# hibikid39/ndt_slam

Hardware: AMD Instinct MI355X
Metric: scan-matches/sec (10k-pt scan vs 1M-pt NDT map) (higher is better)
Workload: dtype f64

## Files before the change

### include/ndt_mi355x.h

```cpp
#ifndef NDT_MI355X_H_
#define NDT_MI355X_H_

#include <stddef.h>
#include <stdint.h>

#ifdef __cplusplus
extern "C" {
#endif

enum ndt_status {
  NDT_OK = 0,
  NDT_E_ARG = -1,
  NDT_E_HIP = -2,
  NDT_E_NO_DEVICE = -3,
  NDT_E_GRID = -4,
  NDT_E_NOMEM = -5
};

typedef struct ndt_params {
  float  resolution;
  double step_size;
  double trans_eps;
  int    max_iter;
  double outlier_ratio;
// ... 25 lines not shown
  int    evals;
  int    ref_evals;
  int    converged;
  int    status;
  int    flags;
  double kbar;
} ndt_result;

enum ndt_result_flags {
  NDT_FLAG_WINDOW_SPILL  = 1,
  NDT_FLAG_REGION_CLIPPED = 2,
  NDT_FLAG_UNSORTED      = 4
};

typedef struct ndt_map_info {
  int min_bx, min_by, div_x, div_y;
  int n_cells;
  int n_valid;
  size_t n_points;
} ndt_map_info;

typedef struct ndt_ctx ndt_ctx;
typedef struct ndt_map ndt_map;

int ndt_default_params(ndt_params *p);
int ndt_params_pcl110(ndt_params *p);
int ndt_params_pcl18(ndt_params *p);
int ndt_params_pcl_new(ndt_params *p);

int ndt_ctx_create(int device, ndt_ctx **out);
int ndt_ctx_destroy(ndt_ctx *ctx);
const char *ndt_last_error(const ndt_ctx *ctx);
void *ndt_ctx_stream(ndt_ctx *ctx);
enum ndt_option { NDT_OPT_MAX_HELPERS = 1, NDT_OPT_WORKGROUPS = 2, NDT_OPT_INJECT_FAULT = 3, NDT_OPT_DEFER_FITNESS = 4 };
int ndt_ctx_set_option(ndt_ctx *ctx, int option, long long value);
int ndt_ctx_set_stream(ndt_ctx *ctx, void *stream);

int ndt_map_build(ndt_ctx *ctx, const float *xy_host, size_t n, size_t stride_bytes,
                  const ndt_params *prm, ndt_map **map);
int ndt_map_build_dev(ndt_ctx *ctx, const float *xy_dev, size_t n, size_t stride_bytes,
                      const ndt_params *prm, ndt_map **map);
#define NDT_REBUILT 1
int ndt_map_rebuild_begin(ndt_ctx *ctx, const float *xy_dev, size_t n, size_t stride_bytes,
                          const ndt_params *prm, ndt_map *map);
int ndt_map_rebuild_end(ndt_ctx *ctx, ndt_map *map);
int ndt_map_destroy(ndt_map *map);
int ndt_map_info_get(const ndt_map *map, ndt_map_info *out);
int ndt_map_export(const ndt_map *map, int *cell_idx, float *cent_xy, double *mean_xy,
                   double *icov_xx_xy_yy, int *npts);

int ndt_align(ndt_ctx *ctx, const ndt_map *map, const float *scan_xy_host, size_t n,
              size_t stride_bytes, const double init_xyyaw[3], ndt_result *out);

int ndt_align_batch(ndt_ctx *ctx, const ndt_map *map, const float *scans_xy_host,
                    const uint64_t *offsets_host, int B, int shared_scan,
                    const double *inits_host , ndt_result *out_host );
int ndt_align_batch_dev(ndt_ctx *ctx, const ndt_map *map, const float *scans_xy_dev,
                        const uint64_t *offsets_dev, int B, size_t total_points, int shared_scan,
                        const double *inits_dev, ndt_result *out_dev, void *stream);
int ndt_align_batch_prepare_dev(ndt_ctx *ctx, const ndt_map *map, const float *scans_xy_dev,
                                const uint64_t *offsets_dev, int B, size_t total_points, int shared_scan,
                                const double *inits_dev, void *stream);
int ndt_prepare_timing(ndt_ctx *ctx, float *order_ms);

int ndt_align_batch_sharded(ndt_ctx *const *ctxs, const ndt_map *const *maps, int n_shards, const float *scans_xy_host,
                            const uint64_t *offsets, int B, int shared_scan, const double *inits_xyyaw,
                            ndt_result *results);
// ... 66 lines not shown
```

### ndt_slam_amd/capi.py

```python
import ctypes as C
import os
import sys

import numpy as np

_HERE = os.path.dirname(os.path.abspath(__file__))
LIB_PATH = os.environ.get("NDT_LIB_PATH") or os.path.join(_HERE, "libndt_mi355x.so")
_LIB = None


class NdtError(RuntimeError):
    pass


class Params(C.Structure):
    _fields_ = [
        ("resolution", C.c_float), ("step_size", C.c_double), ("trans_eps", C.c_double),
        ("max_iter", C.c_int), ("outlier_ratio", C.c_double), ("min_pts", C.c_int),
        ("eig_mult", C.c_double), ("cov_unbiased", C.c_int), ("cov_init_identity", C.c_int),
        ("conv_ge", C.c_int), ("radius_inclusive", C.c_int), ("transform_sse", C.c_int),
        ("stale_h_ang", C.c_int), ("snap_thresh", C.c_double), ("mt_max_iter", C.c_int),
        ("mt_mu", C.c_double), ("mt_nu", C.c_double), ("libm_f32", C.c_int), ("grid_margin", C.c_int),
    ]


class FuseParams(C.Structure):
    _fields_ = [("coe_ndt_cov", C.c_double), ("coe_vel", C.c_double), ("coe_omega", C.c_double),
                ("del_time", C.c_double), ("score_thre", C.c_double)]


class MapInfo(C.Structure):
    _fields_ = [("min_bx", C.c_int), ("min_by", C.c_int), ("div_x", C.c_int), ("div_y", C.c_int),
                ("n_cells", C.c_int), ("n_valid", C.c_int), ("n_points", C.c_size_t)]


RESULT_DTYPE = np.dtype([
    ("pose", "f8", 3), ("T00", "f4"), ("T10", "f4"), ("T03", "f4"), ("T13", "f4"),
    ("fitness", "f8"), ("trans_prob", "f8"), ("score", "f8"), ("H", "f8", 9), ("p", "f8", 3),
    ("iters", "i4"), ("evals", "i4"), ("ref_evals", "i4"), ("converged", "i4"), ("status", "i4"),
    ("flags", "i4"), ("kbar", "f8")], align=True)
RESULT_BYTES = RESULT_DTYPE.itemsize
FLAG_WINDOW_SPILL, FLAG_REGION_CLIPPED, FLAG_UNSORTED = 1, 2, 4
NDT_OK, NDT_E_ARG, NDT_E_HIP, NDT_E_NO_DEVICE, NDT_E_GRID, NDT_E_NOMEM = 0, -1, -2, -3, -4, -5
OPT_MAX_HELPERS, OPT_WORKGROUPS, OPT_INJECT_FAULT, OPT_DEFER_FITNESS = 1, 2, 3, 4

EXPORTS = [
    "ndt_default_params", "ndt_params_pcl110", "ndt_params_pcl18", "ndt_params_pcl_new", "ndt_ctx_create", "ndt_ctx_destroy", "ndt_last_error", "ndt_ctx_stream",
    "ndt_ctx_set_stream", "ndt_ctx_set_option", "ndt_ctx_wait_launch",
    "ndt_map_build", "ndt_map_build_dev", "ndt_map_rebuild_begin", "ndt_map_rebuild_end", "ndt_map_destroy", "ndt_map_info_get", "ndt_map_export",
    "ndt_align", "ndt_align_batch", "ndt_align_batch_dev", "ndt_align_batch_prepare_dev", "ndt_prepare_timing", "ndt_align_batch_trace", "ndt_eval_at",
    "ndt_fitness_at", "ndt_last_timing", "ndt_kernel_timing", "ndt_launch_interval", "ndt_align_batch_sharded", "ndt_prefilter", "ndt_prefilter_batch_dev",
    "ndt_fuse_default_params", "ndt_predict_batch_dev", "ndt_fuse_batch_dev",
    "ndt_remove_neighbors", "ndt_remove_neighbors_dev",
    "ndt_difference_extraction", "ndt_difference_extraction_dev", "ndt_make_map", "ndt_make_map_dev",
    "ndt_selftest_libm_f32",
]


def lib():
    global _LIB
    if _LIB is not None:
        return _LIB
    if not os.path.exists(LIB_PATH):
        raise NdtError("%s is missing: run `python -c 'import __graft_entry__ as g; g.build()'` "
                       "(hipcc --offload-arch=gfx950); there is no CPU fallback" % LIB_PATH)
    L = C.CDLL(LIB_PATH)
    vp, sz, i = C.c_void_p, C.c_size_t, C.c_int
    for name in ("ndt_default_params", "ndt_params_pcl110", "ndt_params_pcl18", "ndt_params_pcl_new"):
        getattr(L, name).argtypes = [C.POINTER(Params)]
    L.ndt_ctx_create.argtypes = [i, C.POINTER(vp)]
    L.ndt_ctx_destroy.argtypes = [vp]
    L.ndt_last_error.restype = C.c_char_p
    L.ndt_last_error.argtypes = [vp]
    L.ndt_ctx_stream.restype = vp
    L.ndt_ctx_stream.argtypes = [vp]
    L.ndt_ctx_set_stream.argtypes = [vp, vp]
    L.ndt_ctx_set_option.argtypes = [vp, i, C.c_longlong]
# ... 325 lines not shown
```

### ndt_slam_amd/csrc/ndt_match.hip.h

```cpp

constexpr int kBlock = 1024;
constexpr int kWaves = kBlock / 64;
#ifndef NDT_KSUB
#define NDT_KSUB 4
#endif
constexpr int kSub = NDT_KSUB;
constexpr int kUnits = kWaves * kSub;
#ifndef NDT_MAX_HELPERS_BUILD
#define NDT_MAX_HELPERS_BUILD 15
#endif
constexpr int kMaxHelpers = NDT_MAX_HELPERS_BUILD;
constexpr int kDefaultHelpers = 8;
constexpr int kBatchHelpers = 2;
#ifndef NDT_IDLE_MAX
#define NDT_IDLE_MAX 800
#endif
#ifndef NDT_XCD_BONUS
#define NDT_XCD_BONUS 6
#endif
#ifndef NDT_NEED_SLOPE
#define NDT_NEED_SLOPE 10
#endif
#ifndef NDT_HELPER_PENALTY
#define NDT_HELPER_PENALTY 12
// ... 98 lines not shown
  int sbox[4];
  int swave[kWaves + 1];
  int sflag[4];
  double wpart[kUnits * 12];
  double wtmp[kWaves * 12];
  double tot[12];
  unsigned long long own_mask;
  unsigned long long hpose[8];
  unsigned long long hword;
  int hrank;
  int jnext;
  int steal;
  unsigned diag[2];
  int clipped;
  MapView M;
  OptParams P;
  const float2 *pts;
  int npts;
  double etab[64];
};

__shared__ Lds g_L;
__shared__ uint4 g_pool[kPoolBytes / 16];

__device__ __forceinline__ Window window_of(const Region &R, const uint4 *pool) {
  Window W;
  W.R = R;
  W.slot = reinterpret_cast<const unsigned short *>(pool);
  W.ent = reinterpret_cast<const CellEntry *>(reinterpret_cast<const char *>(pool) +
                                              ((R.rw * R.rh * 2 + 15) / 16) * 16);
  return W;
}

__device__ __forceinline__ void region_from_bbox(const MapView &M, const Tf32 &T0, Lds &L) {
  {
    Region r = {0, 0, 0, 0, 0, 0};
    L.clipped = 0;
    if (L.sbox[0] <= L.sbox[2]) {
      long long x0 = (long long)L.sbox[0] - kRegionMargin, x1 = (long long)L.sbox[2] + kRegionMargin;
      long long y0 = (long long)L.sbox[1] - kRegionMargin, y1 = (long long)L.sbox[3] + kRegionMargin;
      long long w = x1 - x0 + 1, h = y1 - y0 + 1;
      if (w > 0 && h > 0) {
        if (w * h > kRegionCells) {
          L.clipped = 1;
          const long long w2 = w > 128 ? 128 : w;
          long long h2 = kRegionCells / w2; if (h2 > h) h2 = h;
          const float sx = fminf(fmaxf(floorf(T0.tx * M.inv_leaf), -1.0e9f), 1.0e9f);
          const float sy = fminf(fmaxf(floorf(T0.ty * M.inv_leaf), -1.0e9f), 1.0e9f);
          long long cx0 = ((long long)(int)sx - M.min_bx) - w2 / 2, cy0 = ((long long)(int)sy - M.min_by) - h2 / 2;
          cx0 = cx0 < x0 ? x0 : (cx0 > x1 - w2 + 1 ? x1 - w2 + 1 : cx0);
          cy0 = cy0 < y0 ? y0 : (cy0 > y1 - h2 + 1 ? y1 - h2 + 1 : cy0);
          x0 = cx0; y0 = cy0; w = w2; h = h2;
        }
        const long long far = 1ll << 30;
        x0 = x0 < -far ? -far : (x0 > far ? far : x0); y0 = y0 < -far ? -far : (y0 > far ? far : y0);
        r.x0 = (int)x0; r.y0 = (int)y0; r.rw = (int)w; r.rh = (int)h;
      }
    }
    const int slot_bytes = ((r.rw * r.rh * 2 + 15) / 16) * 16;
    int cap = (kPoolBytes - slot_bytes) / (int)sizeof(CellEntry) - 2;
    r.cap = cap > 0xFFF0 ? 0xFFF0 : cap;
    L.RG = r;
  }
}

template <bool SSE>
__device__ __noinline__ void compute_region(const MapView &M, const Tf32 &T0, const float2 *__restrict__ scan,
// ... 627 lines not shown
    for (; q < q1; ++q) {
      if (lane < 12) dst[(q - q0) * dst_stride + lane] = 0.0;
    }
    if (step != 0 && vtot) {
      const int u = q0 * kWaves + w;
      __builtin_amdgcn_fence(__ATOMIC_RELEASE, "wavefront");
      __builtin_amdgcn_wave_barrier();
      __builtin_amdgcn_fence(__ATOMIC_ACQUIRE, "wavefront");
      if (lane < kUnitWords) {
        const u64 bits = (u64)__double_as_longlong(dst[lane >> 1]);
        st64(&vtot[u * kUnitWords + lane], tag | (u64)(u32)((lane & 1) ? (bits >> 32) : bits));
      }
    }
  }
}

__device__ __forceinline__ bool watchdog(WsHeader *hdr, u64 spin_start, unsigned &polls) {
  if ((++polls & 63u) != 0u) return false;
  if (ld32(&hdr->abort)) return true;
  if (wall_clock64() - spin_start > kWatchTicks) { st32(&hdr->abort, 1u); return true; }
  return false;
}

__device__ __forceinline__ u64 wave_bcast64(u64 v) {
  const u32 lo = __builtin_amdgcn_readfirstlane((u32)v), hi = __builtin_amdgcn_readfirstlane((u32)(v >> 32));
  return ((u64)hi << 32) | lo;
}

struct alignas(16) PrepRec {
  int region[6];
  int clipped, ok;
  AlignState S;
};
constexpr int kPrepWords = (int)(sizeof(PrepRec) / 4);
static_assert(sizeof(PrepRec) % 16 == 0 && kPrepWords <= kBlock, "PrepRec is copied word by word by one workgroup");

template <bool SSE>
__global__ void __launch_bounds__(kBlock)
ndt_order_kernel(MapView M, OptParams P, const float *__restrict__ scans, const unsigned long long *__restrict__ offsets,
                 int B, int shared_scan, const double *__restrict__ inits, float2 *__restrict__ sorted,
                 PrepRec *__restrict__ prep, unsigned *__restrict__ prep_map ) {
  Lds &L = g_L;
  uint4 *const pool = g_pool;
  if (threadIdx.x == 64) { L.M = M; L.P = P; }
  __syncthreads();
  for (int b = (int)blockIdx.x; b < B; b += (int)gridDim.x) {
    const u64 o0 = shared_scan ? offsets[0] : offsets[b];
    const u64 o1 = shared_scan ? offsets[1] : offsets[b + 1];
    const int n = (int)(o1 - o0);
    PrepRec *R = prep + b;
    if (!(n > 0 && n <= kSortRegs)) {
      if (threadIdx.x == 0) R->ok = 0;
      continue;
    }
    const float2 *scan = reinterpret_cast<const float2 *>(scans) + o0;
    float2 *sp = shared_scan ? sorted + (size_t)b * (size_t)n : sorted + o0;
    order_scan_regs<SSE, kSortRegs / kBlock>(L.M, L.P, inits + 3 * (size_t)b, scan, n, L, pool, sp);
    copy_out_ordered(pool, sp, n);
    if (threadIdx.x == 0) {
      const Region r = L.RG;
      R->region[0] = r.x0; R->region[1] = r.y0; R->region[2] = r.rw; R->region[3] = r.rh; R->region[4] = r.cap; R->region[5] = 0;
      R->clipped = L.clipped; R->ok = 1;
    }
    {
      const u32 *src = reinterpret_cast<const u32 *>(&L.S);
      u32 *dst = reinterpret_cast<u32 *>(&R->S);
      if (threadIdx.x < sizeof(AlignState) / 4) dst[threadIdx.x] = src[threadIdx.x];
      const unsigned *wmap = reinterpret_cast<const unsigned *>(L.wpart);
      unsigned *gm = prep_map + (size_t)b * (kRegionCells / 32);
      for (int i = threadIdx.x; i < kRegionCells / 32; i += kBlock) gm[i] = wmap[i];
    }
    __syncthreads();
  }
}

template <bool SSE, bool INCL, bool CHK>
__global__ void __launch_bounds__(kBlock)
ndt_align_kernel(MapView M, OptParams P, const float *__restrict__ scans,
                 const unsigned long long *__restrict__ offsets, int B, int shared_scan,
                 const double *__restrict__ inits, ndt_result *__restrict__ results,
                 double *__restrict__ trace, int trace_cap, int *__restrict__ trace_rows,
                 float2 *__restrict__ sorted ,
                 unsigned char *__restrict__ ws ,
                 int allow_helpers ,
                 unsigned long long *__restrict__ prof ,
                 const PrepRec *__restrict__ prep ,
                 const unsigned *__restrict__ prep_map) {
  Lds &L = g_L;
  uint4 *const pool = g_pool;
  WsHeader *hdr = reinterpret_cast<WsHeader *>(ws);
  ScanCtl *ctl = reinterpret_cast<ScanCtl *>(ws + sizeof(WsHeader));
  u64 *utot = reinterpret_cast<u64 *>(ws + sizeof(WsHeader) + (size_t)B * sizeof(ScanCtl));
  unsigned *wantmap = reinterpret_cast<unsigned *>(ws + sizeof(WsHeader) + (size_t)B * sizeof(ScanCtl) +
                                                  (size_t)B * kUnits * kUnitWords * sizeof(u64));
  const u64 t_start = kProf ? wall_clock64() : 0;
  const int lane = threadIdx.x & 63, wave = threadIdx.x >> 6;
  if (threadIdx.x < 64) L.etab[threadIdx.x] = c_exp2_tab[threadIdx.x];
  if (threadIdx.x == 64) { L.M = M; L.P = P; }
  bool aborted = false;

  int preclaimed = -1;
  int b0 = (int)blockIdx.x;
  if (allow_helpers && B > 0 && B < (int)gridDim.x && blockIdx.x < 4u * (unsigned)B)
// ... 479 lines not shown
```

### ndt_slam_amd/csrc/ndt_mi355x.hip

```cpp

#include <hip/hip_runtime.h>
#include <hip/hip_ext.h>

#include <algorithm>
#include <cfloat>
#include <cmath>
#include <cstdio>
#include <cstdlib>
#include <cstring>
#include <new>
#include <string>
#include <mutex>
#include <set>
#include <utility>
#include <vector>

#include "ndt_mi355x.h"

#pragma clang fp contract(off)

namespace {

thread_local std::string g_last_error;

// ... 86 lines not shown
  PinnedBuf<unsigned> h_bounds;
  std::string err;
  float map_ms = 0.f, align_ms = 0.f;
  DevBuf<unsigned char> d_scan, d_tmp;
  DevBuf<uint64_t> d_off;
  DevBuf<double> d_init, d_trace;
  DevBuf<ndt_result> d_res;
  DevBuf<int> d_rows;
  DevBuf<float> d_fit;
  DevBuf<FitPart> d_fit_part;
  DevBuf<unsigned char> d_far;
  DevBuf<unsigned char> d_pf;
  DevBuf<unsigned char> d_rn;
  DevBuf<unsigned char> d_mm;
  PinnedBuf<unsigned char> h_mm;
  hipEvent_t ev_mm = nullptr; bool mm_pending = false;
  int num_cus = 0;
  int helpers = -1;
  int workgroups = 0;
  int inject_fault = 0;
  struct PrepSet {
    DevBuf<float2> sorted;
    DevBuf<PrepRec> recs;
    DevBuf<unsigned char> maps;
    hipEvent_t ev0 = nullptr, ready = nullptr;
    bool valid = false, timed = false;
    const void *scans = nullptr, *offsets = nullptr, *inits = nullptr, *map = nullptr;
    int B = 0, shared_scan = 0; size_t total_points = 0;
    int min_bx = 0, min_by = 0, div_x = 0, div_y = 0; float inv_leaf = 0.f;
    long long reader = -1;
  } prep[2];
  int prep_last = 1;
  float order_ms = 0.f;
  hipEvent_t ev_scratch = nullptr; hipStream_t scratch_stream = nullptr; bool scratch_used = false, scratch_recorded = false;
  struct LaunchSet { DevBuf<unsigned char> ws; DevBuf<float2> sorted; size_t ws_clean = 0; };
  static constexpr int kDeferSets = 2;
  LaunchSet sets[kDeferSets];
  LaunchRing ring;
  int defer_fitness = 0;
  hipStream_t fit_stream = nullptr;
  struct FitJob {
    MapView V; const float *scans = nullptr; const unsigned long long *offsets = nullptr; int B = 0, shared_scan = 0;
    size_t total_points = 0; float2 *sorted = nullptr; ndt_result *out = nullptr; unsigned char *ws = nullptr;
    size_t zero_bytes = 0, far_cnt_bytes = 0; bool sse = false; hipEvent_t end = nullptr;
  };
  bool deferred_pending = false;
};

struct ndt_map {
  ndt_ctx *ctx = nullptr;
  ndt_params prm;
  ndt_map_info info;
  bool info_valid = false;
  MapView view;
  size_t n = 0, ng = 0, npad = 0;
  DevBuf<int> count, start, npts_grid;
  DevBuf<unsigned long long> scan_state;
  unsigned scan_seq = 0;
  bool count_clean = false;
  DevBuf<int> perm;
  DevBuf<float2> pts, cent;
  DevBuf<double> rec;
  DevBuf<unsigned> bounds; DevBuf<int> counters;
  DevBuf<int> big;
  DevBuf<unsigned> occ;
  DevBuf<unsigned long long> tiles;
  bool pending = false, pend_queued = false;
  const float *pend_xy = nullptr; size_t pend_stride = 0;
  GridDims grid; bool have_grid = false;
  DevBuf<unsigned char> xy_stage;
  std::vector<std::pair<ndt_ctx *, unsigned long long>> readers;
};

namespace {

int fail(ndt_ctx *ctx, int code, const std::string &msg) {
  g_last_error = msg;
  if (ctx) ctx->err = msg;
  return code;
}

struct ScratchScope {
  ndt_ctx *ctx; hipStream_t st; bool is_open = false;
  ScratchScope(ndt_ctx *c, hipStream_t s) : ctx(c), st(s) {}
  ScratchScope(const ScratchScope &) = delete;
  ScratchScope &operator=(const ScratchScope &) = delete;
  int open(bool deferred_launch = false) {
    if (ctx->deferred_pending && !deferred_launch && ctx->ring.launches > 0) {
      HIP_TRY(ctx, hipStreamWaitEvent(st, ctx->ring.end(ctx->ring.launches - 1), 0));
      ctx->deferred_pending = false;
    }
    if (ctx->scratch_used && st != ctx->scratch_stream) {
      if (!ctx->scratch_recorded) HIP_TRY(ctx, hipEventRecord(ctx->ev_scratch, ctx->scratch_stream));
      HIP_TRY(ctx, hipStreamWaitEvent(st, ctx->ev_scratch, 0));
    }
    is_open = true;
    return NDT_OK;
  }
  int close() {
    is_open = false; ctx->scratch_recorded = false;
    if (st != ctx->stream) { HIP_TRY(ctx, hipEventRecord(ctx->ev_scratch, st)); ctx->scratch_recorded = true; }
    ctx->scratch_stream = st; ctx->scratch_used = true;
    return NDT_OK;
  }
// ... 220 lines not shown
}

int ndt_ctx_create(int device, ndt_ctx **out) {
  if (!out) return NDT_E_ARG;
  *out = nullptr;
  int ndev = 0;
  if (hipGetDeviceCount(&ndev) != hipSuccess || ndev <= 0)
    return fail(nullptr, NDT_E_NO_DEVICE, "no HIP device visible: libndt_mi355x has no CPU fallback");
  if (device < 0 || device >= ndev) return fail(nullptr, NDT_E_ARG, "device ordinal out of range");
  ndt_ctx *c = new (std::nothrow) ndt_ctx();
  if (!c) return NDT_E_NOMEM;
  const int rc = ctx_init(c, device);
  if (rc) { ndt_ctx_destroy(c); return rc; }
  { std::lock_guard<std::mutex> lk(g_live_mu); g_live_ctx.insert(c); }
  *out = c;
  return NDT_OK;
}

int ndt_ctx_set_option(ndt_ctx *c, int option, long long value) {
  if (!c) return NDT_E_ARG;
  switch (option) {
    case NDT_OPT_MAX_HELPERS:
      if (value < -1 || value > kMaxHelpers) return fail(c, NDT_E_ARG, "NDT_OPT_MAX_HELPERS: 0 .. 15, or -1 for the default");
      c->helpers = (int)value; return NDT_OK;
    case NDT_OPT_WORKGROUPS:
      if (value < 0 || value > c->num_cus) return fail(c, NDT_E_ARG, "NDT_OPT_WORKGROUPS: 0 (one per CU) .. number of CUs");
      c->workgroups = (int)value; return NDT_OK;
    case NDT_OPT_INJECT_FAULT:
      if (value < 0 || value > 1000000) return fail(c, NDT_E_ARG, "NDT_OPT_INJECT_FAULT: 0 (off) or the number of the launch that fails");
      c->inject_fault = (int)value; return NDT_OK;
    case NDT_OPT_DEFER_FITNESS:
      if (value != 0 && value != 1) return fail(c, NDT_E_ARG, "NDT_OPT_DEFER_FITNESS: 0 or 1");
      c->defer_fitness = (int)value; return NDT_OK;
    default: return fail(c, NDT_E_ARG, "ndt_ctx_set_option: unknown option");
  }
}

int ndt_ctx_destroy(ndt_ctx *c) {
  if (!c) return NDT_E_ARG;
  { std::lock_guard<std::mutex> lk(g_live_mu); g_live_ctx.erase(c); }
  hipError_t e;
  e = hipSetDevice(c->device);
  if (c->stream) e = hipStreamSynchronize(c->stream);
  if (c->fit_stream) { e = hipStreamSynchronize(c->fit_stream); e = hipStreamDestroy(c->fit_stream); }
  if (c->own_stream) e = hipStreamDestroy(c->own_stream);
  if (c->ev0) e = hipEventDestroy(c->ev0);
  if (c->ev1) e = hipEventDestroy(c->ev1);
  if (c->evm0) e = hipEventDestroy(c->evm0);
  if (c->evm1) e = hipEventDestroy(c->evm1);
  if (c->evb) e = hipEventDestroy(c->evb);
  if (c->side) { e = hipStreamSynchronize(c->side); e = hipStreamDestroy(c->side); }
  if (c->ev_fork) e = hipEventDestroy(c->ev_fork);
  if (c->ev_join) e = hipEventDestroy(c->ev_join);
  if (c->ev_mm) e = hipEventDestroy(c->ev_mm);
  if (c->ev_scratch) e = hipEventDestroy(c->ev_scratch);
  for (hipEvent_t r : c->ring.ev) if (r) e = hipEventDestroy(r);
  for (ndt_ctx::PrepSet &S : c->prep) {
    if (S.ready && S.scans) e = hipEventSynchronize(S.ready);
    if (S.ev0) e = hipEventDestroy(S.ev0);
    if (S.ready) e = hipEventDestroy(S.ready);
  }
  (void)e;
  delete c;
  return NDT_OK;
}

// ... 70 lines not shown
  const float inv_leaf = G.inv_leaf;
  const size_t ng = (size_t)G.div_x * G.div_y, npad = (size_t)G.gw * G.gh;
  m->ng = ng; m->npad = npad;
  const int tiles_w = (G.div_x + 7) / 8 + 2, tiles_h = (G.div_y + 7) / 8 + 2;
  const size_t ntile8 = (size_t)tiles_w * tiles_h;

  {
    int rc; bool grown = false;
    const size_t ntiles_ = (ng + kScanTile - 1) / kScanTile;
    if ((rc = m->count.ensure(ctx, ng + 1, &grown))) return rc;
    if (grown) m->count_clean = false;
    if ((rc = m->start.ensure(ctx, ng + 1 + 8))) return rc;
    if ((rc = m->npts_grid.ensure(ctx, ng + 1))) return rc;
    if ((rc = m->scan_state.ensure(ctx, 2 * ntiles_ + 2, &grown))) return rc;
    if (grown)
      HIP_TRY(ctx, hipMemsetAsync(m->scan_state.p, 0, m->scan_state.cap() * sizeof(unsigned long long), st));
    if ((rc = m->perm.ensure(ctx, n + 4))) return rc;
    if ((rc = m->big.ensure(ctx, n / kBigVoxel + 1))) return rc;
    if ((rc = m->occ.ensure(ctx, (ng + 31) / 32 + 2))) return rc;
    if ((rc = m->tiles.ensure(ctx, ntile8))) return rc;
    if ((rc = m->pts.ensure(ctx, n))) return rc;
    if ((rc = m->cent.ensure(ctx, npad))) return rc;
    if ((rc = m->rec.ensure(ctx, npad * 8))) return rc;
  }
  if (!m->count_clean) HIP_TRY(ctx, hipMemsetAsync(m->count.p, 0, m->count.cap() * sizeof(int), st));
  m->count_clean = false;
  if (requeue) {
    HIP_TRY(ctx, hipEventRecord(ctx->ev_fork, st));
    HIP_TRY(ctx, hipStreamWaitEvent(ctx->side, ctx->ev_fork, 0));
  }
  fill_f2_kernel<<<grid_for(npad, 256), 256, 0, ctx->side>>>(m->cent.p, npad, INFINITY, m->tiles.p, ntile8);
  HIP_TRY(ctx, hipEventRecord(ctx->ev_join, ctx->side));

  map_count_kernel<<<grid_for(n, 256), 256, 0, st>>>(xy, stride, n, G, m->count.p, m->counters.p);
  const int ntiles = (int)((ng + kScanTile - 1) / kScanTile);
  int *const start = m->start.p + 4;
  const int big_cap = (int)(n / kBigVoxel + 1);
  m->scan_seq = (m->scan_seq + 1u) & 0x3fffffffu;
  if (m->scan_seq == 0u) m->scan_seq = 1u;
  scan_onepass_kernel<<<ntiles, kScanBlock, 0, st>>>(m->count.p, ng, m->scan_state.p, m->scan_seq, ntiles, m->counters.p + 3, start,
                                                     m->big.p, m->counters.p + 2, big_cap);
  map_scatter_kernel<<<grid_for(n, 256), 256, 0, st>>>(xy, stride, n, G, start, m->count.p, m->perm.p);
  HIP_TRY(ctx, hipGetLastError());
  m->count_clean = true;
  const unsigned small_blocks = (unsigned)((ng + kOrderVoxPerBlock - 1) / kOrderVoxPerBlock);
  map_order_kernel<<<small_blocks + kBigBlocks, 256, 0, st>>>(start, ng, small_blocks, m->big.p, m->counters.p + 2, big_cap, m->perm.p, xy, stride, m->pts.p);
  HIP_TRY(ctx, hipStreamWaitEvent(st, ctx->ev_join, 0));

  LeafParams L;
  L.min_pts = prm->min_pts; L.cov_unbiased = prm->cov_unbiased; L.cov_init_identity = prm->cov_init_identity;
  L.eig_mult = prm->eig_mult;
  hipExtLaunchKernelGGL(map_finalize_kernel, dim3((unsigned)((ng + 255) / 256)), dim3(256), 0, st, nullptr, ctx->evm1, 0, G, L, start,
                        m->pts.p, m->cent.p, m->rec.p, m->npts_grid.p, m->counters.p, m->occ.p, m->tiles.p, tiles_w);
  HIP_TRY(ctx, hipGetLastError());

  MapView &V = m->view;
  V.inv_leaf = inv_leaf; V.leaf = prm->resolution;
  V.r2 = (float)((double)prm->resolution * (double)prm->resolution);
  V.radius_inclusive = prm->radius_inclusive; V.transform_sse = prm->transform_sse;
  V.min_bx = G.min_bx; V.min_by = G.min_by; V.div_x = G.div_x; V.div_y = G.div_y; V.gw = G.gw; V.gh = G.gh;
  V.cent = m->cent.p; V.rec = m->rec.p; V.occ = m->occ.p; V.tiles = m->tiles.p; V.tiles_w = tiles_w; V.pt_start = start; V.pts = m->pts.p;
  gauss_constants(*prm, &V.d1, &V.d2);
  V.e_hi = pair_check_threshold(V.d2);
  m->info.min_bx = G.min_bx; m->info.min_by = G.min_by; m->info.div_x = G.div_x; m->info.div_y = G.div_y;
  m->info.n_points = n;
  return NDT_OK;
}
// ... 183 lines not shown
                   int *npts) {
  if (!cm || !cell_idx || !cent_xy || !mean_xy || !icov || !npts) return NDT_E_ARG;
  ndt_map *m = const_cast<ndt_map *>(cm);
  ndt_ctx *ctx = m->ctx;
  HIP_TRY(ctx, hipSetDevice(ctx->device));
  const size_t ng = m->ng, npad = m->npad;
  int *hn = (int *)malloc(ng * sizeof(int));
  float2 *hc = (float2 *)malloc(npad * sizeof(float2));
  double *hr = (double *)malloc(npad * 8 * sizeof(double));
  if (!hn || !hc || !hr) { free(hn); free(hc); free(hr); return NDT_E_NOMEM; }
  hipError_t e1 = hipMemcpyAsync(hn, m->npts_grid.p, ng * sizeof(int), hipMemcpyDeviceToHost, ctx->stream);
  hipError_t e2 = hipMemcpyAsync(hc, m->cent.p, npad * sizeof(float2), hipMemcpyDeviceToHost, ctx->stream);
  hipError_t e3 = hipMemcpyAsync(hr, m->rec.p, npad * 8 * sizeof(double), hipMemcpyDeviceToHost, ctx->stream);
  hipError_t e4 = hipStreamSynchronize(ctx->stream);
  if (e1 != hipSuccess || e2 != hipSuccess || e3 != hipSuccess || e4 != hipSuccess) {
    free(hn); free(hc); free(hr);
    return fail(ctx, NDT_E_HIP, "ndt_map_export: copy failed");
  }
  size_t k = 0;
  const int gw = m->view.gw, dx = m->view.div_x;
  for (size_t g = 0; g < ng; ++g) {
    if (hn[g] == 0) continue;
    size_t pg = (size_t)(g / dx + 2) * gw + (g % dx + 2);
    cell_idx[k] = (int)g; npts[k] = hn[g];
    cent_xy[2 * k] = hc[pg].x; cent_xy[2 * k + 1] = hc[pg].y;
    mean_xy[2 * k] = hr[pg * 8]; mean_xy[2 * k + 1] = hr[pg * 8 + 1];
    icov[3 * k] = hr[pg * 8 + 2]; icov[3 * k + 1] = hr[pg * 8 + 3]; icov[3 * k + 2] = hr[pg * 8 + 4];
    ++k;
  }
  free(hn); free(hc); free(hr);
  return NDT_OK;
}

int ndt_align_batch_prepare_dev(ndt_ctx *ctx, const ndt_map *map, const float *scans, const uint64_t *offsets,
                                int B, size_t total_points, int shared_scan, const double *inits, void *stream) {
  if (!ctx) return fail(nullptr, NDT_E_ARG, "null context");
  if (!map || !scans || !offsets || !inits || B <= 0 || total_points == 0)
    return fail(ctx, NDT_E_ARG, "ndt_align_batch_prepare_dev: bad arguments");
  if (map->ctx->device != ctx->device) return fail(ctx, NDT_E_ARG, "ndt_align_batch_prepare_dev: the map was built on another device");
  HIP_TRY(ctx, hipSetDevice(ctx->device));
  hipStream_t st = stream ? (hipStream_t)stream : ctx->stream;
  ndt_ctx::PrepSet &S = ctx->prep[ctx->prep_last ^ 1];
  S.valid = false;
  const size_t slots = (shared_scan ? (size_t)B : (size_t)1) * total_points;
  int rc;
  if ((rc = S.sorted.ensure(ctx, slots + 2))) return rc;
  if ((rc = S.recs.ensure(ctx, (size_t)B))) return rc;
  if ((rc = S.maps.ensure(ctx, (size_t)B * (kRegionCells / 8)))) return rc;
  if (!S.ready) { HIP_TRY(ctx, hipEventCreate(&S.ev0)); HIP_TRY(ctx, hipEventCreate(&S.ready)); }
  if (S.reader >= 0 && (unsigned long long)S.reader < ctx->ring.launches)
    HIP_TRY(ctx, hipStreamWaitEvent(st, ctx->ring.end((unsigned long long)S.reader), 0));
  const MapView &V = map->view;
  const OptParams O = opt_of(map->prm);
  const int ncu = ctx->workgroups > 0 ? ctx->workgroups : ctx->num_cus;
  const int grid = B < ncu ? B : ncu;
  if (map->prm.transform_sse)
    hipExtLaunchKernelGGL((ndt_order_kernel<true>), dim3(grid), dim3(kBlock), 0, st, S.ev0, S.ready, 0, V, O, scans,
                          (const unsigned long long *)offsets, B, shared_scan, inits, S.sorted.p, S.recs.p, (unsigned *)S.maps.p);
  else
    hipExtLaunchKernelGGL((ndt_order_kernel<false>), dim3(grid), dim3(kBlock), 0, st, S.ev0, S.ready, 0, V, O, scans,
                          (const unsigned long long *)offsets, B, shared_scan, inits, S.sorted.p, S.recs.p, (unsigned *)S.maps.p);
  HIP_TRY(ctx, hipGetLastError());
  S.scans = scans; S.offsets = offsets; S.inits = inits; S.map = map; S.B = B; S.shared_scan = shared_scan; S.total_points = total_points;
  S.min_bx = V.min_bx; S.min_by = V.min_by; S.div_x = V.div_x; S.div_y = V.div_y; S.inv_leaf = V.inv_leaf;
  S.valid = true; S.timed = false;
  ctx->prep_last ^= 1;
  return NDT_OK;
}

int ndt_align_batch_dev(ndt_ctx *ctx, const ndt_map *map, const float *scans, const uint64_t *offsets,
                        int B, size_t total_points, int shared_scan, const double *inits, ndt_result *out,
                        void *stream) {
  if (!ctx) return fail(nullptr, NDT_E_ARG, "null context");
  if (!map || !scans || !offsets || !inits || !out || B <= 0) return fail(ctx, NDT_E_ARG, "ndt_align_batch: bad arguments");
  if (map->ctx->device != ctx->device) return fail(ctx, NDT_E_ARG, "ndt_align_batch: the map was built on another device");
  if (total_points == 0) return fail(ctx, NDT_E_ARG, "ndt_align_batch: total_points = 0");
  HIP_TRY(ctx, hipSetDevice(ctx->device));
  hipStream_t st = stream ? (hipStream_t)stream : ctx->stream;
  if (st != map->ctx->stream) HIP_TRY(ctx, hipStreamWaitEvent(st, map->ctx->evm1, 0));
  ndt_ctx::PrepSet *pset = nullptr;
  for (ndt_ctx::PrepSet &S : ctx->prep) {
    const MapView &V = map->view;
    if (S.valid && S.scans == scans && S.offsets == offsets && S.inits == inits && S.map == map && S.B == B &&
        S.shared_scan == shared_scan && S.total_points == total_points && S.min_bx == V.min_bx && S.min_by == V.min_by &&
        S.div_x == V.div_x && S.div_y == V.div_y && S.inv_leaf == V.inv_leaf)
      pset = &S;
  }
  if (pset) {
    HIP_TRY(ctx, hipStreamWaitEvent(st, pset->ready, 0));
    pset->valid = false;
  }
  int rc;
  const bool defer = ctx->defer_fitness != 0;
  ScratchScope scope(ctx, st);
  if ((rc = scope.open(defer))) return rc;
  if ((rc = launch_align(ctx, map, st, scans, (const unsigned long long *)offsets, B, shared_scan, total_points, inits,
                         out, nullptr, 0, nullptr, nullptr, pset, defer)))
    return rc;
  return scope.close();
}

int ndt_prepare_timing(ndt_ctx *ctx, float *order_ms) {
  if (!ctx || !order_ms) return NDT_E_ARG;
  *order_ms = 0.f;
  for (ndt_ctx::PrepSet &S : ctx->prep) {
    if (!S.ready || S.reader < 0) continue;
    HIP_TRY(ctx, hipEventSynchronize(S.ready));
    float ms = 0.f;
    HIP_TRY(ctx, hipEventElapsedTime(&ms, S.ev0, S.ready));
    if (ms > *order_ms) *order_ms = ms;
  }
  return NDT_OK;
}

}

namespace {

__global__ void __launch_bounds__(256)
// ... 642 lines not shown
```

Measured before the change: 655,400.

## Rewrite scan ordering kernel as standalone counting sort; add prepare-ahead overlap option

The ordering kernel now uses its own small 256-thread workgroup with private LDS. It does a two-pass bbox and histogram counting sort with wave-level rank computation, launched with one block per scan instead of one per CU. A new opt-in NDT_OPT_PREPARE_AHEAD option queues this ordering on the map's side stream right after the map count kernel, so it can overlap with the rest of the map build. The overlap path is off by default and only fires under narrow conditions (other ctx, B >= CUs), and the rewritten sort adds atomic and serialized per-wave phases.

```diff
diff --git a/include/ndt_mi355x.h b/include/ndt_mi355x.h
--- a/include/ndt_mi355x.h
+++ b/include/ndt_mi355x.h
@@ -81,7 +81,8 @@
 int ndt_ctx_destroy(ndt_ctx *ctx);
 const char *ndt_last_error(const ndt_ctx *ctx);
 void *ndt_ctx_stream(ndt_ctx *ctx);
-enum ndt_option { NDT_OPT_MAX_HELPERS = 1, NDT_OPT_WORKGROUPS = 2, NDT_OPT_INJECT_FAULT = 3, NDT_OPT_DEFER_FITNESS = 4 };
+enum ndt_option { NDT_OPT_MAX_HELPERS = 1, NDT_OPT_WORKGROUPS = 2, NDT_OPT_INJECT_FAULT = 3, NDT_OPT_DEFER_FITNESS = 4,
+                  NDT_OPT_PREPARE_AHEAD = 5 };
 int ndt_ctx_set_option(ndt_ctx *ctx, int option, long long value);
 int ndt_ctx_set_stream(ndt_ctx *ctx, void *stream);
 
diff --git a/ndt_slam_amd/capi.py b/ndt_slam_amd/capi.py
--- a/ndt_slam_amd/capi.py
+++ b/ndt_slam_amd/capi.py
@@ -42,7 +42,7 @@
 RESULT_BYTES = RESULT_DTYPE.itemsize
 FLAG_WINDOW_SPILL, FLAG_REGION_CLIPPED, FLAG_UNSORTED = 1, 2, 4
 NDT_OK, NDT_E_ARG, NDT_E_HIP, NDT_E_NO_DEVICE, NDT_E_GRID, NDT_E_NOMEM = 0, -1, -2, -3, -4, -5
-OPT_MAX_HELPERS, OPT_WORKGROUPS, OPT_INJECT_FAULT, OPT_DEFER_FITNESS = 1, 2, 3, 4
+OPT_MAX_HELPERS, OPT_WORKGROUPS, OPT_INJECT_FAULT, OPT_DEFER_FITNESS, OPT_PREPARE_AHEAD = 1, 2, 3, 4, 5
 
 EXPORTS = [
     "ndt_default_params", "ndt_params_pcl110", "ndt_params_pcl18", "ndt_params_pcl_new", "ndt_ctx_create", "ndt_ctx_destroy", "ndt_last_error", "ndt_ctx_stream",
diff --git a/ndt_slam_amd/csrc/ndt_match.hip.h b/ndt_slam_amd/csrc/ndt_match.hip.h
--- a/ndt_slam_amd/csrc/ndt_match.hip.h
+++ b/ndt_slam_amd/csrc/ndt_match.hip.h
@@ -154,7 +154,8 @@
   return W;
 }
 
-__device__ __forceinline__ void region_from_bbox(const MapView &M, const Tf32 &T0, Lds &L) {
+template <class LdsT>
+__device__ __forceinline__ void region_from_bbox(const MapView &M, const Tf32 &T0, LdsT &L) {
   {
     Region r = {0, 0, 0, 0, 0, 0};
     L.clipped = 0;
@@ -848,16 +849,38 @@
   int clipped, ok;
   AlignState S;
 };
-constexpr int kPrepWords = (int)(sizeof(PrepRec) / 4);
-static_assert(sizeof(PrepRec) % 16 == 0 && kPrepWords <= kBlock, "PrepRec is copied word by word by one workgroup");
+static_assert(sizeof(PrepRec) % 16 == 0, "PrepRec layout");
+
+constexpr int kPrepBlock = 256;
+constexpr int kPrepWaves = kPrepBlock / 64;
+constexpr int kPrepPer = kSortRegs / kBlock;
+constexpr int kPrepHistWords = (kRegionCells + 1 + 1) / 2;
+constexpr int kPrepRunWords = (kPrepHistWords + kPrepBlock - 1) / kPrepBlock;
+static_assert(kSortRegs < 65536 && kSortRegs % kPrepBlock == 0, "u16 counters; whole rounds of sequence numbers");
+
+__host__ __device__ constexpr int prep_point_of_seq(int q) {
+  return ((q >> 6) % kPrepPer) * kBlock + ((q >> 6) / kPrepPer) * 64 + (q & 63);
+}
+
+struct PrepLds {
+  AlignState S;
+  MapView M;
+  OptParams P;
+  Region RG;
+  int sbox[4];
+  int clipped;
+  unsigned wtot[kPrepWaves];
+};
 
 template <bool SSE>
-__global__ void __launch_bounds__(kBlock)
+__global__ void __launch_bounds__(kPrepBlock)
 ndt_order_kernel(MapView M, OptParams P, const float *__restrict__ scans, const unsigned long long *__restrict__ offsets,
                  int B, int shared_scan, const double *__restrict__ inits, float2 *__restrict__ sorted,
                  PrepRec *__restrict__ prep, unsigned *__restrict__ prep_map ) {
-  Lds &L = g_L;
-  uint4 *const pool = g_pool;
+  __shared__ PrepLds L;
+  __shared__ unsigned hist[kPrepHistWords];
+  __shared__ unsigned wmap[kRegionCells / 32];
+  const int wv = (int)(threadIdx.x >> 6), ln = (int)(threadIdx.x & 63);
   if (threadIdx.x == 64) { L.M = M; L.P = P; }
   __syncthreads();
   for (int b = (int)blockIdx.x; b < B; b += (int)gridDim.x) {
@@ -871,20 +894,135 @@
     }
     const float2 *scan = reinterpret_cast<const float2 *>(scans) + o0;
     float2 *sp = shared_scan ? sorted + (size_t)b * (size_t)n : sorted + o0;
-    order_scan_regs<SSE, kSortRegs / kBlock>(L.M, L.P, inits + 3 * (size_t)b, scan, n, L, pool, sp);
-    copy_out_ordered(pool, sp, n);
+    if (threadIdx.x == 0) init_state(L.S, L.P, inits + 3 * (size_t)b, (double)n);
+    if (threadIdx.x == 64) { L.sbox[0] = INT_MAX; L.sbox[1] = INT_MAX; L.sbox[2] = INT_MIN; L.sbox[3] = INT_MIN; }
+    for (int i = threadIdx.x; i < kPrepHistWords; i += kPrepBlock) hist[i] = 0u;
+    for (int i = threadIdx.x; i < kRegionCells / 32; i += kPrepBlock) wmap[i] = 0u;
+    __syncthreads();
+    const Tf32 T0 = L.S.T;
+    const float inv_leaf = L.M.inv_leaf;
+    const int min_bx = L.M.min_bx, min_by = L.M.min_by;
+    auto vox = [&](float2 p, int &ix, int &iy) {
+      float xt, yt;
+      tf_apply_t<SSE>(T0, p.x, p.y, xt, yt);
+      const float fx = fminf(fmaxf(floorf(xt * inv_leaf), -1.0e9f), 1.0e9f);
+      const float fy = fminf(fmaxf(floorf(yt * inv_leaf), -1.0e9f), 1.0e9f);
+      ix = (int)fx - min_bx; iy = (int)fy - min_by;
+      return finite2(xt, yt);
+    };
+    {
+      int mnx = INT_MAX, mny = INT_MAX, mxx = INT_MIN, mxy = INT_MIN;
+      for (int i0 = threadIdx.x; i0 < n; i0 += 4 * kPrepBlock) {
+        float2 p4[4];
+#pragma unroll
+        for (int u = 0; u < 4; ++u) p4[u] = gld_f2(scan + min(i0 + u * kPrepBlock, n - 1));
+#pragma unroll
+        for (int u = 0; u < 4; ++u) {
+          int ix, iy;
+          if (vox(p4[u], ix, iy) && i0 + u * kPrepBlock < n) {
+            mnx = ix < mnx ? ix : mnx; mxx = ix > mxx ? ix : mxx;
+            mny = iy < mny ? iy : mny; mxy = iy > mxy ? iy : mxy;
+          }
+        }
+      }
+      mnx = wave_min_dpp(mnx); mny = wave_min_dpp(mny); mxx = wave_max_dpp(mxx); mxy = wave_max_dpp(mxy);
+      if (ln == 63 && mnx <= mxx) {
+        atomicMin(&L.sbox[0], mnx); atomicMin(&L.sbox[1], mny); atomicMax(&L.sbox[2], mxx); atomicMax(&L.sbox[3], mxy);
+      }
+    }
+    __syncthreads();
+    if (threadIdx.x == 0) region_from_bbox(L.M, L.S.T, L);
+    __syncthreads();
+    const Region r = L.RG;
+    const int ncell = r.rw * r.rh;
+    auto key_of = [&](float2 p) {
+      int ix, iy;
+      const bool fin = vox(p, ix, iy);
+      const int lx = ix - r.x0, ly = iy - r.y0;
+      return (!fin || lx < 0 || lx >= r.rw || ly < 0 || ly >= r.rh) ? ncell : ly * r.rw + lx;
+    };
+    for (int i0 = threadIdx.x; i0 < n; i0 += 4 * kPrepBlock) {
+      float2 p4[4];
+#pragma unroll
+      for (int u = 0; u < 4; ++u) p4[u] = gld_f2(scan + min(i0 + u * kPrepBlock, n - 1));
+#pragma unroll
+      for (int u = 0; u < 4; ++u) {
+        if (i0 + u * kPrepBlock >= n) break;
+        const int k = key_of(p4[u]);
+        atomicAdd(&hist[k >> 1], 1u << ((k & 1) * 16));
+      }
+    }
+    __syncthreads();
+    for (int wi = threadIdx.x; wi < kRegionCells / 32; wi += kPrepBlock) {
+      unsigned bits = 0u;
+#pragma unroll
+      for (int j = 0; j < 16; ++j) {
+        const unsigned h = hist[16 * wi + j];
+        const int c = 32 * wi + 2 * j;
+        bits |= ((h & 0xFFFFu) != 0u && c < ncell) ? 1u << (2 * j) : 0u;
+        bits |= ((h >> 16) != 0u && c + 1 < ncell) ? 1u << (2 * j + 1) : 0u;
+      }
+      wmap[wi] = bits;
+    }
+    {
+      const int w0 = (int)threadIdx.x * kPrepRunWords, w1 = min(w0 + kPrepRunWords, kPrepHistWords);
+      unsigned mine = 0;
+      for (int w = w0; w < w1; ++w) { const unsigned h = hist[w]; mine += (h & 0xFFFFu) + (h >> 16); }
+      const unsigned incl = wave_incl_scan(mine);
+      if (ln == 63) L.wtot[wv] = incl;
+      __syncthreads();
+      unsigned run = incl - mine;
+      for (int w = 0; w < wv; ++w) run += L.wtot[w];
+      for (int w = w0; w < w1; ++w) {
+        const unsigned h = hist[w], lo = h & 0xFFFFu;
+        hist[w] = run | ((run + lo) << 16);
+        run += lo + (h >> 16);
+      }
+    }
+    __syncthreads();
+    float2 nxt = make_float2(0.f, 0.f);
+    {
+      const int i = prep_point_of_seq((int)threadIdx.x);
+      if (i < n) nxt = gld_f2(scan + i);
+    }
+    for (int q0 = 0; q0 < kSortRegs; q0 += kPrepBlock) {
+      const int i = prep_point_of_seq(q0 + (int)threadIdx.x);
+      const bool live = i < n;
+      const float2 pt = nxt;
+      if (q0 + kPrepBlock < kSortRegs) {
+        const int i2 = prep_point_of_seq(q0 + kPrepBlock + (int)threadIdx.x);
+        if (i2 < n) nxt = gld_f2(scan + i2);
+      }
+      const int key = live ? key_of(pt) : -1;
+      int rank = 0, cnt = 0, lead = 63;
+#pragma unroll
+      for (int j = 63; j >= 0; --j) {
+        const bool eq = __builtin_amdgcn_readlane(key, j) == key;
+        rank += (eq && j < ln) ? 1 : 0;
+        cnt += eq ? 1 : 0;
+        lead = eq ? j : lead;
+      }
+      unsigned base = 0u;
+      for (int t = 0; t < kPrepWaves; ++t) {
+        if (wv == t && live && rank == 0) {
+          const int sh = (key & 1) * 16;
+          base = (atomicAdd(&hist[key >> 1], (unsigned)cnt << sh) >> sh) & 0xFFFFu;
+        }
+        sync_lds();
+      }
+      base = (unsigned)__shfl((int)base, lead, 64);
+      if (live) sp[base + rank] = pt;
+    }
     if (threadIdx.x == 0) {
-      const Region r = L.RG;
       R->region[0] = r.x0; R->region[1] = r.y0; R->region[2] = r.rw; R->region[3] = r.rh; R->region[4] = r.cap; R->region[5] = 0;
       R->clipped = L.clipped; R->ok = 1;
     }
     {
       const u32 *src = reinterpret_cast<const u32 *>(&L.S);
       u32 *dst = reinterpret_cast<u32 *>(&R->S);
-      if (threadIdx.x < sizeof(AlignState) / 4) dst[threadIdx.x] = src[threadIdx.x];
-      const unsigned *wmap = reinterpret_cast<const unsigned *>(L.wpart);
+      for (int k = threadIdx.x; k < (int)(sizeof(AlignState) / 4); k += kPrepBlock) dst[k] = src[k];
       unsigned *gm = prep_map + (size_t)b * (kRegionCells / 32);
-      for (int i = threadIdx.x; i < kRegionCells / 32; i += kBlock) gm[i] = wmap[i];
+      for (int k = threadIdx.x; k < kRegionCells / 32; k += kPrepBlock) gm[k] = wmap[k];
     }
     __syncthreads();
   }
diff --git a/ndt_slam_amd/csrc/ndt_mi355x.hip b/ndt_slam_amd/csrc/ndt_mi355x.hip
--- a/ndt_slam_amd/csrc/ndt_mi355x.hip
+++ b/ndt_slam_amd/csrc/ndt_mi355x.hip
@@ -142,6 +142,7 @@
   } prep[2];
   int prep_last = 1;
   float order_ms = 0.f;
+  int prepare_ahead = 0;
   hipEvent_t ev_scratch = nullptr; hipStream_t scratch_stream = nullptr; bool scratch_used = false, scratch_recorded = false;
   struct LaunchSet { DevBuf<unsigned char> ws; DevBuf<float2> sorted; size_t ws_clean = 0; };
   static constexpr int kDeferSets = 2;
@@ -180,6 +181,9 @@
   GridDims grid; bool have_grid = false;
   DevBuf<unsigned char> xy_stage;
   std::vector<std::pair<ndt_ctx *, unsigned long long>> readers;
+  hipEvent_t ev_count = nullptr;
+  unsigned long long builds = 0, prepared_build = 0;
+  ~ndt_map() { if (ev_count) { hipError_t e = hipEventDestroy(ev_count); (void)e; } }
 };
 
 namespace {
@@ -466,6 +470,9 @@
     case NDT_OPT_DEFER_FITNESS:
       if (value != 0 && value != 1) return fail(c, NDT_E_ARG, "NDT_OPT_DEFER_FITNESS: 0 or 1");
       c->defer_fitness = (int)value; return NDT_OK;
+    case NDT_OPT_PREPARE_AHEAD:
+      if (value != 0 && value != 1) return fail(c, NDT_E_ARG, "NDT_OPT_PREPARE_AHEAD: 0 or 1");
+      c->prepare_ahead = (int)value; return NDT_OK;
     default: return fail(c, NDT_E_ARG, "ndt_ctx_set_option: unknown option");
   }
 }
@@ -602,7 +609,10 @@
   fill_f2_kernel<<<grid_for(npad, 256), 256, 0, ctx->side>>>(m->cent.p, npad, INFINITY, m->tiles.p, ntile8);
   HIP_TRY(ctx, hipEventRecord(ctx->ev_join, ctx->side));
 
-  map_count_kernel<<<grid_for(n, 256), 256, 0, st>>>(xy, stride, n, G, m->count.p, m->counters.p);
+  if (!m->ev_count) HIP_TRY(ctx, hipEventCreate(&m->ev_count));
+  hipExtLaunchKernelGGL(map_count_kernel, dim3(grid_for(n, 256)), dim3(256), 0, st, nullptr, m->ev_count, 0,
+                        xy, stride, n, G, m->count.p, m->counters.p);
+  m->builds++;
   const int ntiles = (int)((ng + kScanTile - 1) / kScanTile);
   int *const start = m->start.p + 4;
   const int big_cap = (int)(n / kBigVoxel + 1);
@@ -852,14 +862,12 @@
   return NDT_OK;
 }
 
-int ndt_align_batch_prepare_dev(ndt_ctx *ctx, const ndt_map *map, const float *scans, const uint64_t *offsets,
-                                int B, size_t total_points, int shared_scan, const double *inits, void *stream) {
-  if (!ctx) return fail(nullptr, NDT_E_ARG, "null context");
-  if (!map || !scans || !offsets || !inits || B <= 0 || total_points == 0)
-    return fail(ctx, NDT_E_ARG, "ndt_align_batch_prepare_dev: bad arguments");
-  if (map->ctx->device != ctx->device) return fail(ctx, NDT_E_ARG, "ndt_align_batch_prepare_dev: the map was built on another device");
-  HIP_TRY(ctx, hipSetDevice(ctx->device));
-  hipStream_t st = stream ? (hipStream_t)stream : ctx->stream;
+}
+
+namespace {
+
+int queue_prepare(ndt_ctx *ctx, const ndt_map *map, const float *scans, const uint64_t *offsets, int B, size_t total_points,
+                  int shared_scan, const double *inits, hipStream_t st) {
   ndt_ctx::PrepSet &S = ctx->prep[ctx->prep_last ^ 1];
   S.valid = false;
   const size_t slots = (shared_scan ? (size_t)B : (size_t)1) * total_points;
@@ -872,13 +880,12 @@
     HIP_TRY(ctx, hipStreamWaitEvent(st, ctx->ring.end((unsigned long long)S.reader), 0));
   const MapView &V = map->view;
   const OptParams O = opt_of(map->prm);
-  const int ncu = ctx->workgroups > 0 ? ctx->workgroups : ctx->num_cus;
-  const int grid = B < ncu ? B : ncu;
+  const int grid = B < 65535 ? B : 65535;
   if (map->prm.transform_sse)
-    hipExtLaunchKernelGGL((ndt_order_kernel<true>), dim3(grid), dim3(kBlock), 0, st, S.ev0, S.ready, 0, V, O, scans,
+    hipExtLaunchKernelGGL((ndt_order_kernel<true>), dim3(grid), dim3(kPrepBlock), 0, st, S.ev0, S.ready, 0, V, O, scans,
                           (const unsigned long long *)offsets, B, shared_scan, inits, S.sorted.p, S.recs.p, (unsigned *)S.maps.p);
   else
-    hipExtLaunchKernelGGL((ndt_order_kernel<false>), dim3(grid), dim3(kBlock), 0, st, S.ev0, S.ready, 0, V, O, scans,
+    hipExtLaunchKernelGGL((ndt_order_kernel<false>), dim3(grid), dim3(kPrepBlock), 0, st, S.ev0, S.ready, 0, V, O, scans,
                           (const unsigned long long *)offsets, B, shared_scan, inits, S.sorted.p, S.recs.p, (unsigned *)S.maps.p);
   HIP_TRY(ctx, hipGetLastError());
   S.scans = scans; S.offsets = offsets; S.inits = inits; S.map = map; S.B = B; S.shared_scan = shared_scan; S.total_points = total_points;
@@ -886,6 +893,20 @@
   S.valid = true; S.timed = false;
   ctx->prep_last ^= 1;
   return NDT_OK;
+}
+
+}
+
+extern "C" {
+
+int ndt_align_batch_prepare_dev(ndt_ctx *ctx, const ndt_map *map, const float *scans, const uint64_t *offsets,
+                                int B, size_t total_points, int shared_scan, const double *inits, void *stream) {
+  if (!ctx) return fail(nullptr, NDT_E_ARG, "null context");
+  if (!map || !scans || !offsets || !inits || B <= 0 || total_points == 0)
+    return fail(ctx, NDT_E_ARG, "ndt_align_batch_prepare_dev: bad arguments");
+  if (map->ctx->device != ctx->device) return fail(ctx, NDT_E_ARG, "ndt_align_batch_prepare_dev: the map was built on another device");
+  HIP_TRY(ctx, hipSetDevice(ctx->device));
+  return queue_prepare(ctx, map, scans, offsets, B, total_points, shared_scan, inits, stream ? (hipStream_t)stream : ctx->stream);
 }
 
 int ndt_align_batch_dev(ndt_ctx *ctx, const ndt_map *map, const float *scans, const uint64_t *offsets,
@@ -905,6 +926,15 @@
         S.shared_scan == shared_scan && S.total_points == total_points && S.min_bx == V.min_bx && S.min_by == V.min_by &&
         S.div_x == V.div_x && S.div_y == V.div_y && S.inv_leaf == V.inv_leaf)
       pset = &S;
+  }
+  const int ncu = ctx->workgroups > 0 ? ctx->workgroups : ctx->num_cus;
+  if (!pset && ctx->prepare_ahead && B >= ncu && map->ctx != ctx && map->ev_count && map->builds != map->prepared_build) {
+    hipStream_t side = map->ctx->side;
+    HIP_TRY(ctx, hipStreamWaitEvent(side, map->ev_count, 0));
+    int rc = queue_prepare(ctx, map, scans, offsets, B, total_points, shared_scan, inits, side);
+    if (rc) return rc;
+    const_cast<ndt_map *>(map)->prepared_build = map->builds;
+    pset = &ctx->prep[ctx->prep_last];
   }
   if (pset) {
     HIP_TRY(ctx, hipStreamWaitEvent(st, pset->ready, 0));
```

Result: no change. 654,200, median of 6 (-0.2%).
